# xiaochuanle/MECAT

Measured on AMD Instinct MI355X. Metric: candidate overlaps/sec, higher is better.
Workload: dtype int32

## Files before the change

### mecat_amd/csrc/align.hip

```cpp
#include <stdlib.h>

#include "aln_jobs.h"
#include "dw_defs.h"
#include "scan.h"

__global__ void dw_stitch(const mhip_aln_job* __restrict__ jobs, const DirResult* __restrict__ dres, int n, int min_aln,
                          mhip_aln_result* __restrict__ out, unsigned long long* __restrict__ counters) {
    int i = blockIdx.x * blockDim.x + threadIdx.x;
    if (i >= n) return;
    const DirResult L = dres[2 * i], R = dres[2 * i + 1];
    mhip_aln_result r;
    r.query_start = jobs[i].qstart - L.qbases;
    r.target_start = jobs[i].sstart - L.tbases;
    r.query_end = jobs[i].qstart + R.qbases;
    r.target_end = jobs[i].sstart + R.tbases;
    r.matches = L.matches + R.matches;
    r.columns = L.columns + R.columns;
    r.blocks = L.blocks + R.blocks;
    r.ok = r.columns >= min_aln;
    out[i] = r;
    if (r.ok) {
        atomicAdd(&counters[6], (unsigned long long)(r.query_end - r.query_start));
        atomicAdd(&counters[7], 1ull);
    }
}

__global__ __launch_bounds__(1024) void dw_job_scan(const int32_t* __restrict__ counts, int n_reads, int part_index, int part_count,
                                                    unsigned int* __restrict__ first, int* __restrict__ num_jobs) {
    const unsigned int tot = scan_array_1024<unsigned int>(
        n_reads, 0u, [&](long long i) { return (unsigned int)counts[i]; }, [&](long long i, unsigned int p) { first[i] = p; });
    if (threadIdx.x == 0) {
        unsigned int mine = tot;
        if (part_count > 1) mine = tot / (unsigned)part_count + ((unsigned)part_index < tot % (unsigned)part_count ? 1u : 0u);
        *num_jobs = (int)mine;
    }
}

__global__ __launch_bounds__(256) void dw_make_jobs(const mhip_candidate* __restrict__ cands, const int32_t* __restrict__ counts,
                                                    const unsigned int* __restrict__ first, int n_reads, int maxc, int rid_begin,
                                                    int rid_stride, int ref_start_id, int part_index, int part_count,
                                                    mhip_aln_job* __restrict__ jobs) {
    const size_t t = (size_t)blockIdx.x * blockDim.x + threadIdx.x;
    const int i = (int)(t / (unsigned)maxc), j = (int)(t % (unsigned)maxc);
    if (i >= n_reads || j >= counts[i]) return;
    const unsigned int g = first[i] + (unsigned)j;
    if (part_count > 1 && (int)(g % (unsigned)part_count) != part_index) return;
    const unsigned int slot = part_count > 1 ? g / (unsigned)part_count : g;
    const mhip_candidate cd = cands[(size_t)i * maxc + j];
    mhip_aln_job jb;
    jb.qid_local = rid_begin + i * rid_stride;
    jb.sid_local = cd.readno - ref_start_id;
    jb.chain = cd.chain;
    int qstart = cd.loc2, sstart = cd.loc1;
    if (qstart && sstart) { qstart += MHIP_KMER_SIZE / 2; sstart += MHIP_KMER_SIZE / 2; }
    jb.qstart = qstart;
    jb.sstart = sstart;
    jobs[slot] = jb;
}

int aln_jobs_run(mhip_ctx* c, const mhip_volume* ref, const mhip_volume* reads, const mhip_aln_job* jobs, int n, int min_align_size,
                 mhip_aln_result* out, aln_dev_fn dev) {
    HIPCHK(hipSetDevice(c->device));
    if (n <= 0) return 0;
    char why[96];
    if (aln_jobs_check(jobs, n, reads->h_offs.data(), reads->num_reads, ref->h_offs.data(), ref->num_reads, why, sizeof(why)) >= 0) {
        mhip_set_error("%s", why);
        return -1;
    }
    mhip_aln_job* d_jobs;
    mhip_aln_result* d_out;
    if (c->scratch("al_jobs", sizeof(mhip_aln_job) * (size_t)n, (void**)&d_jobs)) return -1;
    if (c->scratch("al_out", sizeof(mhip_aln_result) * (size_t)n, (void**)&d_out)) return -1;
    HIPCHK(hipMemcpyAsync(d_jobs, jobs, sizeof(mhip_aln_job) * (size_t)n, hipMemcpyHostToDevice, c->stream));
    if (dev(c, ref, reads, d_jobs, n, min_align_size, d_out)) return -1;
    HIPCHK(hipMemcpyAsync(out, d_out, sizeof(mhip_aln_result) * (size_t)n, hipMemcpyDeviceToHost, c->stream));
    HIPCHK(hipStreamSynchronize(c->stream));
    return 0;
}

extern "C" {

int mhip_jobs_from_candidates_dev(mhip_ctx* c, const void* d_cands, const void* d_counts, int n_reads, int maxc, int rid_begin,
                                  int rid_stride, int ref_start_read_id, int part_index, int part_count, void* d_jobs, int* num_jobs) {
    HIPCHK(hipSetDevice(c->device));
    *num_jobs = 0;
    if (n_reads <= 0) return 0;
    if (part_count < 1) part_count = 1;
    int* d_n;
    if (c->scratch("al_njobs", 64, (void**)&d_n)) return -1;
    unsigned int* d_first;
    if (c->scratch("al_jobfirst", sizeof(unsigned int) * (size_t)n_reads, (void**)&d_first)) return -1;
    LAUNCH(c, "dw_job_scan", dw_job_scan, 1, 1024, 0, (const int32_t*)d_counts, n_reads, part_index, part_count, d_first, d_n);
    const size_t nthreads = (size_t)n_reads * (size_t)maxc;
    LAUNCH(c, "dw_make_jobs", dw_make_jobs, (unsigned)((nthreads + 255) / 256), 256, 0, (const mhip_candidate*)d_cands,
           (const int32_t*)d_counts, (const unsigned int*)d_first, n_reads, maxc, rid_begin, rid_stride, ref_start_read_id, part_index,
           part_count, (mhip_aln_job*)d_jobs);
    HIPCHK(hipMemcpyAsync(num_jobs, d_n, sizeof(int), hipMemcpyDeviceToHost, c->stream));
    HIPCHK(hipStreamSynchronize(c->stream));
    return 0;
}

int mhip_align_candidates_dev(mhip_ctx* c, const mhip_volume* ref, const mhip_volume* reads, const void* d_jobs, int n,
                              int min_align_size, void* d_out) {
    HIPCHK(hipSetDevice(c->device));
    if (n <= 0) return 0;
    DirResult* d_dres;
    unsigned int* d_cur;
    if (c->scratch("al_dres", sizeof(DirResult) * 2 * (size_t)n, (void**)&d_dres)) return -1;
    if (c->scratch("al_cursor", 64, (void**)&d_cur)) return -1;
    HIPCHK(hipMemsetAsync(d_cur, 0, 16, c->stream));
    const char* kv = getenv("MECAT_DW_KERNEL");
    if (kv && atoi(kv) == 1) {
        if (dw_extend_launch(c, ref, reads, d_jobs, n, d_dres, nullptr, nullptr, d_cur)) return -1;
    } else {
        DwHandover* d_hand;
        if (c->scratch("al_hand", sizeof(DwHandover) * 2 * (size_t)n, (void**)&d_hand)) return -1;
        if (dw_extend2_launch(c, ref, reads, d_jobs, n, d_dres, d_hand, d_cur + 1, d_cur)) return -1;
        if (dw_extend_launch(c, ref, reads, d_jobs, n, d_dres, d_hand, d_cur + 1, d_cur + 2)) return -1;
    }
    LAUNCH(c, "dw_stitch", dw_stitch, (n + 255) / 256, 256, 0, (const mhip_aln_job*)d_jobs, (const DirResult*)d_dres, n,
           min_align_size, (mhip_aln_result*)d_out, (unsigned long long*)c->d_counters);
    HIPCHK(hipGetLastError());
    return 0;
}

int mhip_align_candidates(mhip_ctx* c, const mhip_volume* ref, const mhip_volume* reads, const mhip_aln_job* jobs, int n,
                          int min_align_size, mhip_aln_result* out) {
    return aln_jobs_run(c, ref, reads, jobs, n, min_align_size, out, mhip_align_candidates_dev);
}

}
```

### mecat_amd/csrc/aln_jobs.h

```cpp
#pragma once
#include <stddef.h>
#include <stdio.h>

#include "mecat_hip.h"

inline int aln_jobs_check(const mhip_aln_job* jobs, int n, const mhip_offset_t* q_offs, int q_reads, const mhip_offset_t* s_offs, int s_reads,
                          char* msg, size_t msg_cap) {
    for (int i = 0; i < n; ++i) {
        const mhip_aln_job& j = jobs[i];
        if (j.qid_local < 0 || j.qid_local >= q_reads || j.sid_local < 0 || j.sid_local >= s_reads) {
            snprintf(msg, msg_cap, "alignment job %d: read index out of range", i);
            return i;
        }
        if (j.qstart > q_offs[(size_t)j.qid_local].size || j.sstart > s_offs[(size_t)j.sid_local].size) {
            snprintf(msg, msg_cap, "alignment job %d: start point outside the reads", i);
            return i;
        }
    }
    return -1;
}

typedef int (*aln_dev_fn)(mhip_ctx* c, const mhip_volume* ref, const mhip_volume* reads, const void* d_jobs, int n, int min_align_size, void* d_out);

int aln_jobs_run(mhip_ctx* c, const mhip_volume* ref, const mhip_volume* reads, const mhip_aln_job* jobs, int n, int min_align_size,
                 mhip_aln_result* out, aln_dev_fn dev);
```

### mecat_amd/csrc/dw_defs.h

```cpp
#pragma once
#include "common.h"

#define AL_BLOCK 256
#define AL_WAVES (AL_BLOCK / WAVE)
#define SEG_BLK 500

struct DirResult {
    int32_t qbases, tbases, matches, columns, blocks, pad;
};

struct DwHandover {
    uint32_t unit;
    int32_t qidx, tidx;
    DirResult R;
};

int dw_extend2_launch(mhip_ctx* c, const mhip_volume* ref, const mhip_volume* reads, const void* d_jobs, int n, DirResult* dres,
                      DwHandover* hand, unsigned int* hand_count, unsigned int* cursor);
int dw_extend_launch(mhip_ctx* c, const mhip_volume* ref, const mhip_volume* reads, const void* d_jobs, int n, DirResult* dres,
                     const DwHandover* hand, const unsigned int* hand_count, unsigned int* cursor);
```

### mecat_amd/csrc/dw_extend.hip

```cpp
#include <stdlib.h>

#include <algorithm>

#include "dw_defs.h"

#define MAX_BLK 736
#define SEQ_WORDS 52
#define MAX_D 400
#define VU_LEN (2 * MAX_D + 8)
#define ROW_W 224
#define RING 16
#define GROW_STRIDE ((size_t)MAX_D * ROW_W + 2 * (MAX_D + 8))

struct AlnWaveLds {
    uint32_t Qp[SEQ_WORDS];
    uint32_t Tp[SEQ_WORDS];
    int16_t V[VU_LEN];
    uint16_t ring[RING * ROW_W];
    int16_t rmin[RING];
    int16_t rmax[RING];
};

#include "dw_helpers.h"

// ... 148 lines not shown
            switch (nj) {
            case 1: row_body<1, SPILL>(S, grow, lane, d, nslot, min_k, max_k, k_offset, q_len, t_len, best_m, band_tol, snake, bkey, hkey, x0); break;
            case 2: row_body<2, SPILL>(S, grow, lane, d, nslot, min_k, max_k, k_offset, q_len, t_len, best_m, band_tol, snake, bkey, hkey, x0); break;
            case 3: row_body<3, SPILL>(S, grow, lane, d, nslot, min_k, max_k, k_offset, q_len, t_len, best_m, band_tol, snake, bkey, hkey, x0); break;
            default: row_body<4, SPILL>(S, grow, lane, d, nslot, min_k, max_k, k_offset, q_len, t_len, best_m, band_tol, snake, bkey, hkey, x0); break;
            }
            xreg = x0;
        }
        bkey = __builtin_amdgcn_readfirstlane(bkey);
        hkey = __builtin_amdgcn_readfirstlane(hkey);
        reg_ok = nj == 1;
        reg_min_k = min_k;
        st.rows += 1; st.fast_rows += fast ? 1u : 0u; st.wide_rows += nj > 1 ? 1u : 0u;
        cells += (unsigned int)nslot;
        {
            const int rm = bkey >> 10, rk = 1023 - (bkey & 1023) - k_offset;
            if (rm > best_m) { best_m = rm; best_x = (rm + rk) / 2; best_y = best_x - rk; best_d = d; best_k = rk; }
        }
        int nmin, nmax;
        bool whole = false;
        if (fast) {
            const int m0 = __builtin_amdgcn_readlane(mreg, 0), ml = __builtin_amdgcn_readlane(mreg, nslot - 1);
            whole = m0 >= best_m - band_tol && ml >= best_m - band_tol;
        }
        if (whole) { nmin = min_k; nmax = max_k; }
        else band_keys<SPILL>(S, lane, nj, nslot, min_k, max_k, k_offset, best_m, band_tol, nmin, nmax);
        max_k = __builtin_amdgcn_readfirstlane(nmax) + 1;
        min_k = __builtin_amdgcn_readfirstlane(nmin) - 1;
        __builtin_amdgcn_wave_barrier();
        if (hkey != 0x7fffffff) {
            aligned = 1; end_k = (hkey >> 10) - k_offset; end_x = hkey & 1023; end_y = end_x - end_k; end_d = d;
            break;
        }
    }
    o.trim_ok = 0; o.qcnt = o.tcnt = o.acnt = 0;
    if (!aligned) {
        st.unaligned += 1;
        if (best_x > 0) { end_x = best_x; end_y = best_y; end_d = best_d; end_k = best_k; }
        else { o.aligned_or_best = 0; o.qe = o.te = o.dist = 0; return; }
    }
    o.aligned_or_best = 1; o.qe = end_x; o.te = end_y; o.dist = end_d;
    const int aln_size = (end_x + end_y + end_d) / 2;
    int cd = end_d, ck = end_k, cx2 = end_x;
    int qcnt = 0, tcnt = 0, acnt = 0, found = 0;
    while (true) {
        int x1, pre_k = 0, takes_q = 0;
        if (cd == 0) x1 = 0;
        else {
            if (!SPILL && last_row - (cd - 1) >= RING) { o.fallback = 1; return; }
            int pmin, pmax, cmin, cmax, vl = 0, vr = 0;
            const int kl = ck - 1, kr = ck + 1;
            if (SPILL) {
                pmin = g_rmin[cd - 1]; pmax = g_rmax[cd - 1]; cmin = g_rmin[cd]; cmax = g_rmax[cd];
                const uint16_t* prow = grow + (size_t)(cd - 1) * ROW_W;
                if (kl >= pmin && kl <= pmax) vl = prow[(kl - pmin) >> 1];
                if (kr >= pmin && kr <= pmax) vr = prow[(kr - pmin) >> 1];
            } else {
                pmin = S.rmin[(cd - 1) % RING]; pmax = S.rmax[(cd - 1) % RING]; cmin = S.rmin[cd % RING]; cmax = S.rmax[cd % RING];
                const uint16_t* prow = S.ring + ((cd - 1) % RING) * ROW_W;
                if (kl >= pmin && kl <= pmax) vl = prow[(kl - pmin) >> 1];
                if (kr >= pmin && kr <= pmax) vr = prow[(kr - pmin) >> 1];
            }
            if (ck == cmin || (ck != cmax && vl < vr)) { x1 = vr; pre_k = kr; takes_q = 0; }
            else { x1 = vl + 1; pre_k = kl; takes_q = 1; }
        }
        const int s = cx2 - x1;
        if (s >= 4) { acnt += 4; qcnt += 4; tcnt += 4; found = 1; break; }
        acnt += s; qcnt += s; tcnt += s;
        if (cd == 0) break;
        acnt += 1;
        if (takes_q) { qcnt += 1; cx2 = x1 - 1; } else { tcnt += 1; cx2 = x1; }
        ck = pre_k;
        --cd;
    }
    o.qcnt = qcnt; o.tcnt = tcnt; o.acnt = acnt;
    o.trim_ok = found && (aln_size - acnt >= 2);
}

__global__ __launch_bounds__(AL_BLOCK) void dw_extend(const uint32_t* __restrict__ rpac, const mhip_offset_t* __restrict__ roffs,
                                                      const uint32_t* __restrict__ qpac, const mhip_offset_t* __restrict__ qoffs,
                                                      const mhip_aln_job* __restrict__ jobs, int n, DirResult* __restrict__ dres,
                                                      uint16_t* __restrict__ gscratch, unsigned int* __restrict__ cursor,
                                                      unsigned long long* __restrict__ counters, const DwHandover* __restrict__ hand,
                                                      const unsigned int* __restrict__ hand_count) {
    __shared__ AlnWaveLds lds[AL_WAVES];
    AlnWaveLds& S = lds[threadIdx.x >> 6];
    const int lane = lane_id();
    const int gw = blockIdx.x * AL_WAVES + (threadIdx.x >> 6);
    uint16_t* grow = gscratch + (size_t)gw * GROW_STRIDE;
    unsigned long long cells = 0, snake = 0, nblocks = 0, nfallback = 0;
    unsigned int ucells = 0, usnake = 0;
    DwStats st = {0, 0, 0, 0, 0};
    while (true) {
        unsigned int unit = 0;
        if (lane == 0) unit = atomicAdd(cursor, 1u);
        unit = __shfl(unit, 0);
        int qidx = 0, tidx = 0;
        DirResult R = {0, 0, 0, 0, 0, 0};
        if (hand) {
            if (unit >= *hand_count) break;
            const DwHandover h = hand[unit];
            unit = h.unit; qidx = h.qidx; tidx = h.tidx; R = h.R;
        } else if (unit >= 2u * (unsigned)n) break;
        const mhip_aln_job jb = jobs[unit >> 1];
        const int right = unit & 1;
        const int qsize = qoffs[jb.qid_local].size, tsize = roffs[jb.sid_local].size;
        SeqView q, t;
        q.pac = qpac; q.off = qoffs[jb.qid_local].offset; q.comp = jb.chain;
        t.pac = rpac; t.off = roffs[jb.sid_local].offset; t.comp = 0;
        int query_size, target_size;
        const int qs0 = right ? jb.qstart : jb.qstart - 1, step = right ? 1 : -1;
        if (jb.chain) { q.A = qsize - 1 - qs0; q.B = -step; } else { q.A = qs0; q.B = step; }
        t.A = right ? jb.sstart : jb.sstart - 1; t.B = step;
        if (right) { query_size = qsize - jb.qstart; target_size = tsize - jb.sstart; }
        else { query_size = jb.qstart; target_size = jb.sstart; }
        if (jb.qstart < 0 || jb.sstart < 0) { query_size = 0; target_size = 0; }
        while (true) {
            const int qleft = query_size - qidx, tleft = target_size - tidx;
            int qblk, tblk, last_block;
            if (qleft < SEG_BLK + 100 || tleft < SEG_BLK + 100) {
                qblk = min(qleft, (int)(tleft + tleft * 0.2));
                tblk = min(tleft, (int)(qleft + qleft * 0.2));
                last_block = 1;
            } else { qblk = SEG_BLK; tblk = SEG_BLK; last_block = 0; }
            if (qblk < 0) qblk = 0;
            if (tblk < 0) tblk = 0;
            __builtin_amdgcn_wave_barrier();
            if (lane < SEQ_WORDS) {
                S.Qp[lane] = (lane > 0 && (lane - 1) * 16 < qblk + 32) ? view_word(q, qidx + (lane - 1) * 16) : 0u;
                S.Tp[lane] = (lane > 0 && (lane - 1) * 16 < tblk + 32) ? view_word(t, tidx + (lane - 1) * 16) : 0u;
            }
            __builtin_amdgcn_wave_barrier();
            BlockOut o;
            align_block<false>(S, qblk, tblk, grow, o, ucells, usnake, st);
            if (o.fallback) { ++nfallback; align_block<true>(S, qblk, tblk, grow, o, ucells, usnake, st); }
            ++nblocks;
            R.blocks += 1;
            if (!o.aligned_or_best || !o.trim_ok) break;
            const int full_map = (qblk - o.qe <= 20 || tblk - o.te <= 20);
            int qcnt = o.qcnt, tcnt = o.tcnt, acnt = o.acnt;
            if (last_block || !full_map) { qcnt -= 4; tcnt -= 4; acnt -= 4; }
            const int cols = (o.qe + o.te + o.dist) / 2 - acnt;
            const int mcut = qcnt + tcnt - acnt;
            R.columns += cols;
            R.matches += (o.qe + o.te - o.dist) / 2 - mcut;
            R.qbases += o.qe - qcnt;
            R.tbases += o.te - tcnt;
            if (last_block || !full_map) break;
            qidx += o.qe - qcnt;
            tidx += o.te - tcnt;
        }
        if (lane == 0) dres[unit] = R;
        cells += ucells; snake += usnake;
        ucells = 0; usnake = 0;
    }
    for (int off = 32; off > 0; off >>= 1) snake += __shfl_xor(snake, off);
    if (lane == 0) {
        atomicAdd(&counters[3], nblocks);
        atomicAdd(&counters[4], cells);
        atomicAdd(&counters[5], snake);
        atomicAdd(&counters[8], nfallback);
        atomicAdd(&counters[9], (unsigned long long)st.rows);
        atomicAdd(&counters[10], (unsigned long long)st.fast_rows);
        atomicAdd(&counters[11], (unsigned long long)st.wide_rows);
        atomicAdd(&counters[12], (unsigned long long)st.unaligned);
    }
}

int dw_extend_launch(mhip_ctx* c, const mhip_volume* ref, const mhip_volume* reads, const void* d_jobs, int n, DirResult* dres,
                     const DwHandover* hand, const unsigned int* hand_count, unsigned int* cursor) {
    int waves_per_cu = 16;
    if (const char* e = getenv("MECAT_DW_WAVES")) waves_per_cu = std::max(4, std::min(32, atoi(e)));
    const int max_waves = c->num_cus * waves_per_cu;
    const int grid = std::min(max_waves / AL_WAVES, (2 * n + AL_WAVES - 1) / AL_WAVES);
    uint16_t* d_g;
    if (c->scratch("al_rows", sizeof(uint16_t) * GROW_STRIDE * (size_t)max_waves, (void**)&d_g)) return -1;
    LAUNCH(c, "dw_extend", dw_extend, grid, AL_BLOCK, 0, (const uint32_t*)ref->d_pac, (const mhip_offset_t*)ref->d_offs,
           (const uint32_t*)reads->d_pac, (const mhip_offset_t*)reads->d_offs, (const mhip_aln_job*)d_jobs, n, dres, d_g, cursor,
           (unsigned long long*)c->d_counters, hand, hand_count);
    return 0;
}
```

### mecat_amd/csrc/xalign.hip

```cpp
#include <stdlib.h>

#include <algorithm>
#include <type_traits>

#include "aln_jobs.h"
#include "common.h"
#include "xd_defs.h"
#include "xd_block_ring.h"
#include "xd_block_wide.h"

template <bool WIDE>
__global__ __launch_bounds__(XW_BLOCK, 6) void xd_extend_w(const uint32_t* __restrict__ rpac, const mhip_offset_t* __restrict__ roffs,
                                                        const uint32_t* __restrict__ qpac, const mhip_offset_t* __restrict__ qoffs,
                                                        const mhip_aln_job* __restrict__ jobs, int n, XDir* __restrict__ dres,
                                                        uint8_t* __restrict__ scratch, unsigned int* __restrict__ cursor,
                                                        unsigned int* __restrict__ ovf_list, unsigned long long* __restrict__ counters,
                                                        const unsigned int* __restrict__ ulist, unsigned int nunits,
                                                        uint8_t* __restrict__ wide_state, const unsigned int* __restrict__ order) {
    __shared__ typename std::conditional<WIDE, XwWide, XrLds>::type lds[WIDE ? 1 : XW_WAVES];
    auto& S = lds[threadIdx.x >> 6];
    const int lane = lane_id();
    uint8_t* st = scratch + (size_t)(blockIdx.x * (blockDim.x >> 6) + (threadIdx.x >> 6)) * (WIDE ? XW_WIDE_BYTES : XR_STATE_BYTES);
    uint8_t* wst = WIDE ? nullptr : wide_state + (size_t)(blockIdx.x * (blockDim.x >> 6) + (threadIdx.x >> 6)) * XW_INPLACE_BYTES;
    unsigned long long nblocks = 0, ncells = 0, nrows = 0, nredone = 0;
// ... 107 lines not shown
    mhip_aln_result r;
    r.query_start = jobs[i].qstart - L.qbases;
    r.target_start = jobs[i].sstart - L.tbases;
    r.query_end = jobs[i].qstart + R.qbases;
    r.target_end = jobs[i].sstart + R.tbases;
    r.matches = L.matches + R.matches;
    r.columns = L.columns + R.columns;
    r.blocks = L.blocks + R.blocks;
    r.ok = (r.query_end - r.query_start) >= min_aln;
    out[i] = r;
    if (r.ok) {
        atomicAdd(&counters[6], (unsigned long long)(r.query_end - r.query_start));
        atomicAdd(&counters[7], 1ull);
    }
}

struct XdMode {
    bool all_wide;
    bool handover;
    bool order;
    int waves_per_cu;
};
static XdMode xd_mode() {
    auto is = [](const char* name, int v) { const char* s = getenv(name); return s && atoi(s) == v; };
    XdMode m;
    m.all_wide = is("MECAT_XD_WIDE", 1);
    m.handover = is("MECAT_XD_HANDOVER", 1);
    m.order = !is("MECAT_XD_ORDER", 0);
    m.waves_per_cu = getenv("MECAT_XW_WAVES") ? atoi(getenv("MECAT_XW_WAVES")) : 24;
    return m;
}

static int xd_launch_ring(mhip_ctx* c, const mhip_volume* ref, const mhip_volume* reads, const void* d_jobs, int n, bool handover, int waves,
                          XDir* d_dres, unsigned int* d_cur, unsigned int* d_ovf, const unsigned int* d_order, unsigned int* nwide) {
    const int grid = std::min(waves / XW_WAVES, (2 * n + XW_WAVES - 1) / XW_WAVES);
    const size_t launched = (size_t)grid * XW_WAVES;
    uint8_t *d_s, *d_wst = nullptr;
    if (c->scratch("xw_state", XR_STATE_BYTES * launched, (void**)&d_s)) return -1;
    if (!handover && c->scratch("xw_inplace", XW_INPLACE_BYTES * launched, (void**)&d_wst)) return -1;
    LAUNCH(c, "xd_extend_w", xd_extend_w<false>, grid, XW_BLOCK, 0, (const uint32_t*)ref->d_pac, (const mhip_offset_t*)ref->d_offs,
           (const uint32_t*)reads->d_pac, (const mhip_offset_t*)reads->d_offs, (const mhip_aln_job*)d_jobs, n, d_dres, d_s, d_cur,
           d_ovf, (unsigned long long*)c->d_counters, (const unsigned int*)nullptr, 2u * (unsigned)n, d_wst, d_order);
    HIPCHK(hipMemcpyAsync(nwide, d_ovf, sizeof(unsigned int), hipMemcpyDeviceToHost, c->stream));
    HIPCHK(hipStreamSynchronize(c->stream));
    if (getenv("MECAT_TRACE")) {
        if (d_wst) {
            unsigned long long redone = 0;
            HIPCHK(hipMemcpy(&redone, (unsigned long long*)c->d_counters + 33, sizeof(redone), hipMemcpyDeviceToHost));
            fprintf(stderr, "[mecat_hip] X-drop: %d units, %llu blocks so far redone in place with the wide window\n", 2 * n, redone);
        } else fprintf(stderr, "[mecat_hip] X-drop: %u of %d units need the wide-window path\n", *nwide, 2 * n);
    }
    return 0;
}

static int xd_launch_wide(mhip_ctx* c, const mhip_volume* ref, const mhip_volume* reads, const void* d_jobs, int n, XDir* d_dres,
                          unsigned int* d_cur, unsigned int* d_ovf, const unsigned int* ulist, unsigned int nu) {
    const int wgrid = (int)std::min(nu, 2048u);
    uint8_t* d_w;
    if (c->scratch("xw_wide", XW_WIDE_BYTES * (size_t)wgrid, (void**)&d_w)) return -1;
    LAUNCH(c, "xd_extend_wide", xd_extend_w<true>, wgrid, 64, 0, (const uint32_t*)ref->d_pac, (const mhip_offset_t*)ref->d_offs,
           (const uint32_t*)reads->d_pac, (const mhip_offset_t*)reads->d_offs, (const mhip_aln_job*)d_jobs, n, d_dres, d_w, d_cur + 2,
           d_ovf + 6 * (size_t)n + 4, (unsigned long long*)c->d_counters, ulist, nu, (uint8_t*)nullptr, (const unsigned int*)nullptr);
    return 0;
}

extern "C" {

int mhip_xalign_candidates_dev(mhip_ctx* c, const mhip_volume* ref, const mhip_volume* reads, const void* d_jobs, int n,
                               int min_align_size, void* d_out) {
    HIPCHK(hipSetDevice(c->device));
    if (n <= 0) return 0;
    const XdMode mode = xd_mode();
    XDir* d_dres;
    unsigned int *d_cur, *d_ovf;
    if (c->scratch("xa_dres", sizeof(XDir) * 2 * (size_t)n, (void**)&d_dres)) return -1;
    if (c->scratch("xa_cursor", 64, (void**)&d_cur)) return -1;
    if (c->scratch("xa_ovf", sizeof(unsigned int) * (6 * (size_t)n + 8), (void**)&d_ovf)) return -1;
    HIPCHK(hipMemsetAsync(d_cur, 0, 16, c->stream));
    unsigned int nwide = 0;
    if (!mode.all_wide) {
        const int waves = c->num_cus * mode.waves_per_cu;
        HIPCHK(hipMemsetAsync(d_ovf, 0, sizeof(unsigned int), c->stream));
        unsigned int* d_order = nullptr;
        if (mode.order && xd_order_jobs(c, ref, reads, d_jobs, n, waves, &d_order)) return -1;
        if (xd_launch_ring(c, ref, reads, d_jobs, n, mode.handover, waves, d_dres, d_cur, d_ovf, d_order, &nwide)) return -1;
    }
    if (nwide > 0 || mode.all_wide) {
        const unsigned int* ulist = mode.all_wide ? nullptr : d_ovf + 1;
        if (xd_launch_wide(c, ref, reads, d_jobs, n, d_dres, d_cur, d_ovf, ulist, mode.all_wide ? 2u * (unsigned)n : nwide)) return -1;
    }
    LAUNCH(c, "xd_stitch", xd_stitch, (n + 255) / 256, 256, 0, (const mhip_aln_job*)d_jobs, (const XDir*)d_dres, n, min_align_size,
           (mhip_aln_result*)d_out, (unsigned long long*)c->d_counters);
    HIPCHK(hipStreamSynchronize(c->stream));
    HIPCHK(hipGetLastError());
    return 0;
}

int mhip_xalign_candidates(mhip_ctx* c, const mhip_volume* ref, const mhip_volume* reads, const mhip_aln_job* jobs, int n,
                           int min_align_size, mhip_aln_result* out) {
    return aln_jobs_run(c, ref, reads, jobs, n, min_align_size, out, mhip_xalign_candidates_dev);
}

}
```

### mecat_amd/csrc/xd_defs.h

```cpp
#pragma once
#include "common.h"

#define X_SEG 500
#define X_MAXN 736
#define X_MIN_SCORE (-100000000)

enum { XS_SUB = 3, XS_GAP_IN_A = 0, XS_GAP_IN_B = 6, XS_OP_MASK = 0x07, XS_EXT_A = 0x10, XS_EXT_B = 0x40 };

struct XDir {
    int32_t qbases, tbases, matches, columns;
    int32_t last_q, last_t, last_m;
    int32_t blocks;
};

struct XView {
    const uint32_t* pac;
    int64_t off;
    int A, B, comp;
};
__device__ __forceinline__ int xv_at(const XView& v, int i) {
    const uint32_t c = pac_base(v.pac, v.off + v.A + (int64_t)v.B * i);
    return (int)(v.comp ? 3u - c : c);
}

// ... 32 lines not shown
    int m = 0, found = 0;
    int want_l1 = 0, first = 0, l1 = 0;
    int sn_n = 0, sn_a = 0, sn_b = 0, sn_m = 0;

    __device__ __forceinline__ void column_type(int pk) {
        first = n == 0 ? pk : first;
        l1 = want_l1 ? pk : l1;
        want_l1 = 0;
    }
    __device__ __forceinline__ void step(int cq, int ct, int cm, int a_after, int b_after) {
        column_type(cq | (ct << 1) | (cm << 2));
        ++n;
        nmatch += cm;
        m = cm ? m + 1 : 0;
        if (m == 4 && !found) { found = 1; want_l1 = 1; sn_n = n; sn_a = a_after; sn_b = b_after; sn_m = nmatch; }
    }
    __device__ __forceinline__ void run(int r, uint32_t Mbits, int a_before, int b_before) {
        const uint32_t mask = r >= 32 ? 0xffffffffu : ((1u << r) - 1u);
        const uint32_t inv = ~Mbits & mask;
        if (!found) {
            const int z = inv ? __builtin_ctz(inv) : r;
            int hit = -1;
            if (m + z >= 4) hit = 3 - m;
            else {
                const uint32_t Q = Mbits & (Mbits >> 1) & (Mbits >> 2) & (Mbits >> 3);
                if (Q) hit = __builtin_ctz(Q) + 3;
            }
            if (hit >= 0) {
                found = 1;
                sn_n = n + hit + 1; sn_a = a_before - (hit + 1); sn_b = b_before - (hit + 1);
                sn_m = nmatch + __builtin_popcount(Mbits & ((2u << hit) - 1u));
                if (hit + 1 < r) l1 = 3 | (int)(((Mbits >> (hit + 1)) & 1u) << 2);
                else want_l1 = 1;
            }
        }
        m = inv ? r - 1 - (31 - __builtin_clz(inv)) : m + r;
    }
    __device__ __forceinline__ void gap_after_run(int gq, int gt) {
        l1 = want_l1 ? (gq | (gt << 1)) : l1;
        want_l1 = 0;
        m = 0;
        ++n;
    }
    __device__ __forceinline__ void finish(int ae, int be, XBlockOut& o) const {
        o.n = n; o.nmatch = nmatch;
        o.l0q = first & 1; o.l0t = (first >> 1) & 1; o.l0m = first >> 2;
        o.l1q = l1 & 1; o.l1t = (l1 >> 1) & 1; o.l1m = l1 >> 2;
        o.acnt = found ? sn_n : n; o.qcnt = found ? ae - sn_a : ae; o.tcnt = found ? be - sn_b : be; o.mtail = found ? sn_m : nmatch;
        o.trim_ok = found && (n - o.acnt >= 2);
    }
};

#define XW_WAVES 4
#define XW_BLOCK (XW_WAVES * 64)
#define XW_RING 128
#define XW_ROWCELLS 128
#define XW_WIN 4096
#define XW_WSTRIDE 768
#define XW_WIDE_BYTES ((size_t)(X_MAXN + 2) * XW_WSTRIDE)
#define XW_WIDE_HF (X_MAXN + 8)
#define XW_INPLACE_STATE 16384
#define XW_INPLACE_BYTES (XW_INPLACE_STATE + XW_WIDE_BYTES)
#define XW_NEG (-(1 << 30))
#define XS_MATCH 0x80
static_assert(XW_ROWCELLS <= XW_RING, "a row's script cells are cells of the ring");
static_assert(XW_WSTRIDE >= X_MAXN + 1 && XW_WIDE_HF >= X_MAXN + 1, "a wide row and the wide score array hold every cell of a block");
static_assert(XW_WIN % 256 == 0, "the wide traceback's window is loaded in rounds of one dword per lane");

template <int CTRL, int RMASK> __device__ __forceinline__ int xw_dpp_max(int v) {
    return max(v, __builtin_amdgcn_update_dpp((int)0x80000000, v, CTRL, RMASK, 0xf, false));
}
__device__ __forceinline__ int xw_scan_max(int v) {
    v = xw_dpp_max<0x111, 0xf>(v);
    v = xw_dpp_max<0x112, 0xf>(v);
    v = xw_dpp_max<0x114, 0xf>(v);
    v = xw_dpp_max<0x118, 0xf>(v);
    v = xw_dpp_max<0x142, 0xa>(v);
    v = xw_dpp_max<0x143, 0xc>(v);
    return v;
}
__device__ __forceinline__ int xw_shr1(int v, int fill) {
    return __builtin_amdgcn_update_dpp(fill, v, 0x138, 0xf, 0xf, false);
}

int xd_order_jobs(mhip_ctx* c, const mhip_volume* ref, const mhip_volume* reads, const void* d_jobs, int n, int waves, unsigned int** d_order);
```

### mecat_amd/csrc/xd_order.hip

```cpp
#include <algorithm>

#include "common.h"
#include "scan.h"
#include "xd_defs.h"

#define XO_BINS 64
__device__ __forceinline__ int xo_bin(const mhip_aln_job& jb, const mhip_offset_t* __restrict__ roffs, const mhip_offset_t* __restrict__ qoffs) {
    int reach = 0;
    if (jb.qstart >= 0 && jb.sstart >= 0) {
        const int qsize = qoffs[jb.qid_local].size, tsize = roffs[jb.sid_local].size;
        reach = max(min(qsize - jb.qstart, tsize - jb.sstart), min(jb.qstart, jb.sstart));
    }
    return XO_BINS - 1 - min(max(reach, 0) >> 10, XO_BINS - 1);
}
#define XO_THREADS 256
template <bool PLACE>
__global__ __launch_bounds__(XO_THREADS) void xo_order_jobs(const mhip_aln_job* __restrict__ jobs, int n, const mhip_offset_t* __restrict__ roffs,
                                                          const mhip_offset_t* __restrict__ qoffs, unsigned int* __restrict__ cnt, unsigned int* __restrict__ order) {
    __shared__ uint16_t tc[XO_BINS][XO_THREADS];
    __shared__ unsigned int wsum[XO_THREADS / 64];
    __shared__ unsigned int base;
    const int t = (int)threadIdx.x, G = (int)gridDim.x;
    const int per_block = (n + G - 1) / G, b0 = min(n, (int)blockIdx.x * per_block), b1 = min(n, b0 + per_block);
    const int per = (b1 - b0 + XO_THREADS - 1) / XO_THREADS, lo = min(b1, b0 + t * per), hi = min(b1, lo + per);
    for (int b = 0; b < XO_BINS; ++b) tc[b][t] = 0;
    for (int i = lo; i < hi; ++i) ++tc[xo_bin(jobs[i], roffs, qoffs)][t];
    __syncthreads();
    unsigned int mypos[XO_BINS];
#pragma unroll
    for (int b = 0; b < XO_BINS; ++b) {
        if (t == 0) base = PLACE ? cnt[(size_t)b * G + blockIdx.x] : 0u;
        const unsigned int c = tc[b][t];
        unsigned int incl = c;
        for (int o = 1; o < 64; o <<= 1) {
            const unsigned int v = __shfl_up(incl, o);
            if ((t & 63) >= o) incl += v;
        }
        if ((t & 63) == 63) wsum[t >> 6] = incl;
        __syncthreads();
        unsigned int before = base;
        for (int k = 0; k < (t >> 6); ++k) before += wsum[k];
        mypos[b] = before + incl - c;
        if (!PLACE && t == XO_THREADS - 1) cnt[(size_t)b * G + blockIdx.x] = before + incl;
        __syncthreads();
    }
    if (!PLACE) return;
    for (int i = lo; i < hi; ++i) {
        const int b = xo_bin(jobs[i], roffs, qoffs);
        unsigned int p = 0;
#pragma unroll
        for (int k = 0; k < XO_BINS; ++k) if (k == b) p = mypos[k]++;
        order[p] = (unsigned int)i;
    }
}
__global__ __launch_bounds__(1024) void xo_scan(unsigned int* __restrict__ cnt, int m) {
    scan_array_1024<unsigned int>(m, 0u, [&](long long i) { return cnt[i]; }, [&](long long i, unsigned int p) { cnt[i] = p; });
}

int xd_order_jobs(mhip_ctx* c, const mhip_volume* ref, const mhip_volume* reads, const void* d_jobs, int n, int waves, unsigned int** d_order) {
    *d_order = nullptr;
    if ((size_t)n <= (size_t)waves) return 0;
    const int G = (int)std::min<size_t>((size_t)c->num_cus, ((size_t)n + 4095) / 4096 + 1);
    unsigned int *d_cnt, *d_ord;
    if (c->scratch("xo_cnt", sizeof(unsigned int) * XO_BINS * (size_t)G, (void**)&d_cnt)) return -1;
    if (c->scratch("xo_order", sizeof(unsigned int) * (size_t)n, (void**)&d_ord)) return -1;
    if ((size_t)n / ((size_t)G * XO_THREADS) >= 65535) return 0;
    LAUNCH(c, "xo_count", xo_order_jobs<false>, G, XO_THREADS, 0, (const mhip_aln_job*)d_jobs, n, (const mhip_offset_t*)ref->d_offs, (const mhip_offset_t*)reads->d_offs, d_cnt, d_ord);
    LAUNCH(c, "xo_scan", xo_scan, 1, 1024, 0, d_cnt, XO_BINS * G);
    LAUNCH(c, "xo_place", xo_order_jobs<true>, G, XO_THREADS, 0, (const mhip_aln_job*)d_jobs, n, (const mhip_offset_t*)ref->d_offs, (const mhip_offset_t*)reads->d_offs, d_cnt, d_ord);
    *d_order = d_ord;
    return 0;
}
```

Measured before the change: 7.067 million.

## Order DW jobs and handover units longest-first and run handover blocks directly

Reuses the xd binning sort, moved to a shared file, to reorder alignment jobs by estimated reach, longest first. The jobs are permuted before the two-stage extend kernels, and results are scattered back to the original order in stitch. The handover units for the second kernel are also bin-sorted by remaining distance in a single-block kernel. Handover blocks now skip the fast-path attempt and go straight to the full-row alignment. The aim is to cut tail imbalance across waves and avoid redundant fast-path attempts that would fall back anyway, at the cost of extra sort and permute kernels.

```diff
diff --git a/mecat_amd/csrc/align.hip b/mecat_amd/csrc/align.hip
--- a/mecat_amd/csrc/align.hip
+++ b/mecat_amd/csrc/align.hip
@@ -1,11 +1,19 @@
 #include <stdlib.h>
+
+#include <algorithm>
 
 #include "aln_jobs.h"
 #include "dw_defs.h"
 #include "scan.h"
 
+__global__ void dw_permute_jobs(const mhip_aln_job* __restrict__ jobs, const unsigned int* __restrict__ order, int n,
+                                mhip_aln_job* __restrict__ ordered) {
+    const int p = blockIdx.x * blockDim.x + threadIdx.x;
+    if (p < n) ordered[p] = jobs[order[p]];
+}
+
 __global__ void dw_stitch(const mhip_aln_job* __restrict__ jobs, const DirResult* __restrict__ dres, int n, int min_aln,
-                          mhip_aln_result* __restrict__ out, unsigned long long* __restrict__ counters) {
+                          mhip_aln_result* __restrict__ out, unsigned long long* __restrict__ counters, const unsigned int* __restrict__ order) {
     int i = blockIdx.x * blockDim.x + threadIdx.x;
     if (i >= n) return;
     const DirResult L = dres[2 * i], R = dres[2 * i + 1];
@@ -18,7 +26,7 @@
     r.columns = L.columns + R.columns;
     r.blocks = L.blocks + R.blocks;
     r.ok = r.columns >= min_aln;
-    out[i] = r;
+    out[order ? order[i] : (unsigned int)i] = r;
     if (r.ok) {
         atomicAdd(&counters[6], (unsigned long long)(r.query_end - r.query_start));
         atomicAdd(&counters[7], 1ull);
@@ -110,16 +118,28 @@
     if (c->scratch("al_cursor", 64, (void**)&d_cur)) return -1;
     HIPCHK(hipMemsetAsync(d_cur, 0, 16, c->stream));
     const char* kv = getenv("MECAT_DW_KERNEL");
+    unsigned int* d_order = nullptr;
     if (kv && atoi(kv) == 1) {
-        if (dw_extend_launch(c, ref, reads, d_jobs, n, d_dres, nullptr, nullptr, d_cur)) return -1;
+        if (dw_extend_launch(c, ref, reads, d_jobs, n, d_dres, nullptr, nullptr, d_cur, nullptr)) return -1;
     } else {
         DwHandover* d_hand;
         if (c->scratch("al_hand", sizeof(DwHandover) * 2 * (size_t)n, (void**)&d_hand)) return -1;
+        const char* ov = getenv("MECAT_DW_ORDER");
+        const int order_mode = ov ? atoi(ov) : 1;
+        int waves_per_cu = DW2_WAVES_PER_SIMD * 4;
+        if (const char* e = getenv("MECAT_DW_WAVES")) waves_per_cu = std::max(4, std::min(32, atoi(e)));
+        if (order_mode != 0 && aln_order_jobs(c, ref, reads, d_jobs, n, order_mode == 2 ? 0 : c->num_cus * waves_per_cu, &d_order)) return -1;
+        if (d_order) {
+            mhip_aln_job* d_ordered;
+            if (c->scratch("al_jobs_ordered", sizeof(mhip_aln_job) * (size_t)n, (void**)&d_ordered)) return -1;
+            LAUNCH(c, "dw_permute_jobs", dw_permute_jobs, (n + 255) / 256, 256, 0, (const mhip_aln_job*)d_jobs, (const unsigned int*)d_order, n, d_ordered);
+            d_jobs = d_ordered;
+        }
         if (dw_extend2_launch(c, ref, reads, d_jobs, n, d_dres, d_hand, d_cur + 1, d_cur)) return -1;
-        if (dw_extend_launch(c, ref, reads, d_jobs, n, d_dres, d_hand, d_cur + 1, d_cur + 2)) return -1;
+        if (dw_extend_launch(c, ref, reads, d_jobs, n, d_dres, d_hand, d_cur + 1, d_cur + 2, d_cur + 3)) return -1;
     }
     LAUNCH(c, "dw_stitch", dw_stitch, (n + 255) / 256, 256, 0, (const mhip_aln_job*)d_jobs, (const DirResult*)d_dres, n,
-           min_align_size, (mhip_aln_result*)d_out, (unsigned long long*)c->d_counters);
+           min_align_size, (mhip_aln_result*)d_out, (unsigned long long*)c->d_counters, (const unsigned int*)d_order);
     HIPCHK(hipGetLastError());
     return 0;
 }
diff --git a/mecat_amd/csrc/aln_jobs.h b/mecat_amd/csrc/aln_jobs.h
--- a/mecat_amd/csrc/aln_jobs.h
+++ b/mecat_amd/csrc/aln_jobs.h
@@ -20,6 +20,8 @@
     return -1;
 }
 
+int aln_order_jobs(mhip_ctx* c, const mhip_volume* ref, const mhip_volume* reads, const void* d_jobs, int n, int waves, unsigned int** d_order);
+
 typedef int (*aln_dev_fn)(mhip_ctx* c, const mhip_volume* ref, const mhip_volume* reads, const void* d_jobs, int n, int min_align_size, void* d_out);
 
 int aln_jobs_run(mhip_ctx* c, const mhip_volume* ref, const mhip_volume* reads, const mhip_aln_job* jobs, int n, int min_align_size,
diff --git a/mecat_amd/csrc/aln_order.hip b/mecat_amd/csrc/aln_order.hip
--- /dev/null
+++ b/mecat_amd/csrc/aln_order.hip
@@ -0,0 +1,73 @@
+#include <algorithm>
+
+#include "aln_jobs.h"
+#include "common.h"
+#include "scan.h"
+
+#define XO_BINS 64
+__device__ __forceinline__ int xo_bin(const mhip_aln_job& jb, const mhip_offset_t* __restrict__ roffs, const mhip_offset_t* __restrict__ qoffs) {
+    int reach = 0;
+    if (jb.qstart >= 0 && jb.sstart >= 0) {
+        const int qsize = qoffs[jb.qid_local].size, tsize = roffs[jb.sid_local].size;
+        reach = max(min(qsize - jb.qstart, tsize - jb.sstart), min(jb.qstart, jb.sstart));
+    }
+    return XO_BINS - 1 - min(max(reach, 0) >> 10, XO_BINS - 1);
+}
+#define XO_THREADS 256
+template <bool PLACE>
+__global__ __launch_bounds__(XO_THREADS) void xo_order_jobs(const mhip_aln_job* __restrict__ jobs, int n, const mhip_offset_t* __restrict__ roffs,
+                                                          const mhip_offset_t* __restrict__ qoffs, unsigned int* __restrict__ cnt, unsigned int* __restrict__ order) {
+    __shared__ uint16_t tc[XO_BINS][XO_THREADS];
+    __shared__ unsigned int wsum[XO_THREADS / 64];
+    __shared__ unsigned int base;
+    const int t = (int)threadIdx.x, G = (int)gridDim.x;
+    const int per_block = (n + G - 1) / G, b0 = min(n, (int)blockIdx.x * per_block), b1 = min(n, b0 + per_block);
+    const int per = (b1 - b0 + XO_THREADS - 1) / XO_THREADS, lo = min(b1, b0 + t * per), hi = min(b1, lo + per);
+    for (int b = 0; b < XO_BINS; ++b) tc[b][t] = 0;
+    for (int i = lo; i < hi; ++i) ++tc[xo_bin(jobs[i], roffs, qoffs)][t];
+    __syncthreads();
+    unsigned int mypos[XO_BINS];
+#pragma unroll
+    for (int b = 0; b < XO_BINS; ++b) {
+        if (t == 0) base = PLACE ? cnt[(size_t)b * G + blockIdx.x] : 0u;
+        const unsigned int c = tc[b][t];
+        unsigned int incl = c;
+        for (int o = 1; o < 64; o <<= 1) {
+            const unsigned int v = __shfl_up(incl, o);
+            if ((t & 63) >= o) incl += v;
+        }
+        if ((t & 63) == 63) wsum[t >> 6] = incl;
+        __syncthreads();
+        unsigned int before = base;
+        for (int k = 0; k < (t >> 6); ++k) before += wsum[k];
+        mypos[b] = before + incl - c;
+        if (!PLACE && t == XO_THREADS - 1) cnt[(size_t)b * G + blockIdx.x] = before + incl;
+        __syncthreads();
+    }
+    if (!PLACE) return;
+    for (int i = lo; i < hi; ++i) {
+        const int b = xo_bin(jobs[i], roffs, qoffs);
+        unsigned int p = 0;
+#pragma unroll
+        for (int k = 0; k < XO_BINS; ++k) if (k == b) p = mypos[k]++;
+        order[p] = (unsigned int)i;
+    }
+}
+__global__ __launch_bounds__(1024) void xo_scan(unsigned int* __restrict__ cnt, int m) {
+    scan_array_1024<unsigned int>(m, 0u, [&](long long i) { return cnt[i]; }, [&](long long i, unsigned int p) { cnt[i] = p; });
+}
+
+int aln_order_jobs(mhip_ctx* c, const mhip_volume* ref, const mhip_volume* reads, const void* d_jobs, int n, int waves, unsigned int** d_order) {
+    *d_order = nullptr;
+    if ((size_t)n <= (size_t)waves) return 0;
+    const int G = (int)std::min<size_t>((size_t)c->num_cus, ((size_t)n + 4095) / 4096 + 1);
+    unsigned int *d_cnt, *d_ord;
+    if (c->scratch("xo_cnt", sizeof(unsigned int) * XO_BINS * (size_t)G, (void**)&d_cnt)) return -1;
+    if (c->scratch("xo_order", sizeof(unsigned int) * (size_t)n, (void**)&d_ord)) return -1;
+    if ((size_t)n / ((size_t)G * XO_THREADS) >= 65535) return 0;
+    LAUNCH(c, "xo_count", xo_order_jobs<false>, G, XO_THREADS, 0, (const mhip_aln_job*)d_jobs, n, (const mhip_offset_t*)ref->d_offs, (const mhip_offset_t*)reads->d_offs, d_cnt, d_ord);
+    LAUNCH(c, "xo_scan", xo_scan, 1, 1024, 0, d_cnt, XO_BINS * G);
+    LAUNCH(c, "xo_place", xo_order_jobs<true>, G, XO_THREADS, 0, (const mhip_aln_job*)d_jobs, n, (const mhip_offset_t*)ref->d_offs, (const mhip_offset_t*)reads->d_offs, d_cnt, d_ord);
+    *d_order = d_ord;
+    return 0;
+}
diff --git a/mecat_amd/csrc/dw_defs.h b/mecat_amd/csrc/dw_defs.h
--- a/mecat_amd/csrc/dw_defs.h
+++ b/mecat_amd/csrc/dw_defs.h
@@ -17,5 +17,12 @@
 
 int dw_extend2_launch(mhip_ctx* c, const mhip_volume* ref, const mhip_volume* reads, const void* d_jobs, int n, DirResult* dres,
                       DwHandover* hand, unsigned int* hand_count, unsigned int* cursor);
+#ifndef DW2_WAVES_PER_SIMD
+#define DW2_WAVES_PER_SIMD 8
+#endif
 int dw_extend_launch(mhip_ctx* c, const mhip_volume* ref, const mhip_volume* reads, const void* d_jobs, int n, DirResult* dres,
-                     const DwHandover* hand, const unsigned int* hand_count, unsigned int* cursor);
+                     const DwHandover* hand, const unsigned int* hand_count, unsigned int* cursor, unsigned int* hand_sorted);
+
+#define DW_SLOT_RERUN 46
+#define DW_SLOT_DIRECT 47
+#define DW_SLOT_DEALT 48
diff --git a/mecat_amd/csrc/dw_extend.hip b/mecat_amd/csrc/dw_extend.hip
--- a/mecat_amd/csrc/dw_extend.hip
+++ b/mecat_amd/csrc/dw_extend.hip
@@ -254,13 +254,14 @@
                                                       const mhip_aln_job* __restrict__ jobs, int n, DirResult* __restrict__ dres,
                                                       uint16_t* __restrict__ gscratch, unsigned int* __restrict__ cursor,
                                                       unsigned long long* __restrict__ counters, const DwHandover* __restrict__ hand,
-                                                      const unsigned int* __restrict__ hand_count) {
+                                                      const unsigned int* __restrict__ hand_count, const unsigned int* __restrict__ hand_order,
+                                                      const unsigned int* __restrict__ hand_sorted, int hand_direct) {
     __shared__ AlnWaveLds lds[AL_WAVES];
     AlnWaveLds& S = lds[threadIdx.x >> 6];
     const int lane = lane_id();
     const int gw = blockIdx.x * AL_WAVES + (threadIdx.x >> 6);
     uint16_t* grow = gscratch + (size_t)gw * GROW_STRIDE;
-    unsigned long long cells = 0, snake = 0, nblocks = 0, nfallback = 0;
+    unsigned long long cells = 0, snake = 0, nblocks = 0, nfallback = 0, ndirect = 0, ndealt = 0;
     unsigned int ucells = 0, usnake = 0;
     DwStats st = {0, 0, 0, 0, 0};
     while (true) {
@@ -269,10 +270,14 @@
         unit = __shfl(unit, 0);
         int qidx = 0, tidx = 0;
         DirResult R = {0, 0, 0, 0, 0, 0};
+        bool keep_rows = false;
         if (hand) {
             if (unit >= *hand_count) break;
-            const DwHandover h = hand[unit];
+            const bool sorted = *hand_sorted != 0u;
+            const DwHandover h = hand[sorted ? hand_order[unit] : unit];
+            ndealt += sorted ? 1u : 0u;
             unit = h.unit; qidx = h.qidx; tidx = h.tidx; R = h.R;
+            keep_rows = hand_direct != 0;
         } else if (unit >= 2u * (unsigned)n) break;
         const mhip_aln_job jb = jobs[unit >> 1];
         const int right = unit & 1;
@@ -304,8 +309,13 @@
             }
             __builtin_amdgcn_wave_barrier();
             BlockOut o;
-            align_block<false>(S, qblk, tblk, grow, o, ucells, usnake, st);
-            if (o.fallback) { ++nfallback; align_block<true>(S, qblk, tblk, grow, o, ucells, usnake, st); }
+            if (keep_rows) ++ndirect;
+            else {
+                align_block<false>(S, qblk, tblk, grow, o, ucells, usnake, st);
+                if (o.fallback) { ++nfallback; keep_rows = true; }
+            }
+            if (keep_rows) align_block<true>(S, qblk, tblk, grow, o, ucells, usnake, st);
+            keep_rows = false;
             ++nblocks;
             R.blocks += 1;
             if (!o.aligned_or_best || !o.trim_ok) break;
@@ -331,7 +341,9 @@
         atomicAdd(&counters[3], nblocks);
         atomicAdd(&counters[4], cells);
         atomicAdd(&counters[5], snake);
-        atomicAdd(&counters[8], nfallback);
+        atomicAdd(&counters[DW_SLOT_RERUN], nfallback);
+        atomicAdd(&counters[DW_SLOT_DIRECT], ndirect);
+        atomicAdd(&counters[DW_SLOT_DEALT], ndealt);
         atomicAdd(&counters[9], (unsigned long long)st.rows);
         atomicAdd(&counters[10], (unsigned long long)st.fast_rows);
         atomicAdd(&counters[11], (unsigned long long)st.wide_rows);
@@ -339,16 +351,91 @@
     }
 }
 
+#define HO_BINS 64
+#define HO_THREADS 256
+#define HO_MAX 65536
+__global__ __launch_bounds__(HO_THREADS) void dw_hand_order(const DwHandover* __restrict__ hand, const unsigned int* __restrict__ hand_count,
+                                                            const mhip_aln_job* __restrict__ jobs, const mhip_offset_t* __restrict__ roffs,
+                                                            const mhip_offset_t* __restrict__ qoffs, unsigned int max_sorted,
+                                                            uint8_t* __restrict__ keys, unsigned int* __restrict__ order,
+                                                            unsigned int* __restrict__ sorted) {
+    __shared__ uint16_t tc[HO_BINS][HO_THREADS];
+    __shared__ unsigned int bin_first[HO_BINS];
+    const unsigned int cnt = *hand_count;
+    if (cnt < 2u || cnt > max_sorted) return;
+    const int t = (int)threadIdx.x, w = t >> 6, l = t & 63;
+    for (int b = 0; b < HO_BINS; ++b) tc[b][t] = 0;
+#pragma unroll 4
+    for (unsigned int i = t; i < cnt; i += HO_THREADS) {
+        const unsigned int unit = hand[i].unit;
+        const int qidx = hand[i].qidx, tidx = hand[i].tidx;
+        const mhip_aln_job jb = jobs[unit >> 1];
+        int rest = 0;
+        if (jb.qstart >= 0 && jb.sstart >= 0) {
+            const int qsize = qoffs[jb.qid_local].size, tsize = roffs[jb.sid_local].size;
+            rest = (unit & 1u) ? min(qsize - jb.qstart - qidx, tsize - jb.sstart - tidx) : min(jb.qstart - qidx, jb.sstart - tidx);
+        }
+        const int b = HO_BINS - 1 - min(max(rest, 0) >> 10, HO_BINS - 1);
+        keys[i] = (uint8_t)b;
+    }
+    __syncthreads();
+    const unsigned int per = (cnt + HO_THREADS - 1) / HO_THREADS, lo = min(cnt, t * per), hi = min(cnt, lo + per);
+    for (unsigned int i = lo; i < hi; ++i) ++tc[keys[i]][t];
+    __syncthreads();
+    for (int b = w; b < HO_BINS; b += HO_THREADS / 64) {
+        unsigned int c[4], sum = 0;
+        for (int k = 0; k < 4; ++k) { c[k] = tc[b][4 * l + k]; sum += c[k]; }
+        unsigned int incl = sum;
+        for (int o = 1; o < 64; o <<= 1) {
+            const unsigned int v = __shfl_up(incl, o);
+            if (l >= o) incl += v;
+        }
+        unsigned int before = incl - sum;
+        for (int k = 0; k < 4; ++k) { tc[b][4 * l + k] = (uint16_t)before; before += c[k]; }
+        if (l == 63) bin_first[b] = incl;
+    }
+    __syncthreads();
+    if (t < HO_BINS) {
+        const unsigned int cb = bin_first[t];
+        unsigned int incl = cb;
+        for (int o = 1; o < 64; o <<= 1) {
+            const unsigned int v = __shfl_up(incl, o);
+            if (l >= o) incl += v;
+        }
+        bin_first[t] = incl - cb;
+    }
+    __syncthreads();
+    for (unsigned int i = lo; i < hi; ++i) {
+        const int b = keys[i];
+        order[bin_first[b] + tc[b][t]++] = i;
+    }
+    if (t == 0) *sorted = 1u;
+}
+
 int dw_extend_launch(mhip_ctx* c, const mhip_volume* ref, const mhip_volume* reads, const void* d_jobs, int n, DirResult* dres,
-                     const DwHandover* hand, const unsigned int* hand_count, unsigned int* cursor) {
+                     const DwHandover* hand, const unsigned int* hand_count, unsigned int* cursor, unsigned int* hand_sorted) {
     int waves_per_cu = 16;
     if (const char* e = getenv("MECAT_DW_WAVES")) waves_per_cu = std::max(4, std::min(32, atoi(e)));
     const int max_waves = c->num_cus * waves_per_cu;
     const int grid = std::min(max_waves / AL_WAVES, (2 * n + AL_WAVES - 1) / AL_WAVES);
     uint16_t* d_g;
     if (c->scratch("al_rows", sizeof(uint16_t) * GROW_STRIDE * (size_t)max_waves, (void**)&d_g)) return -1;
+    const char* e = getenv("MECAT_DW_HAND_DIRECT");
+    const int hand_direct = hand && !(e && atoi(e) == 0);
+    unsigned int* d_ord = nullptr;
+    if (hand) {
+        e = getenv("MECAT_DW_HAND_SORT_MAX");
+        const size_t max_sorted = std::min<size_t>(e ? (size_t)std::max(0, atoi(e)) : (size_t)HO_MAX, (size_t)HO_MAX);
+        const size_t cap = std::max<size_t>(std::min<size_t>(2 * (size_t)n, max_sorted), 1);
+        uint8_t* d_keys;
+        if (c->scratch("al_handord", sizeof(unsigned int) * cap, (void**)&d_ord)) return -1;
+        if (c->scratch("al_handkey", cap, (void**)&d_keys)) return -1;
+        if (max_sorted >= 2)
+            LAUNCH(c, "dw_hand_order", dw_hand_order, 1, HO_THREADS, 0, hand, hand_count, (const mhip_aln_job*)d_jobs,
+                   (const mhip_offset_t*)ref->d_offs, (const mhip_offset_t*)reads->d_offs, (unsigned int)max_sorted, d_keys, d_ord, hand_sorted);
+    }
     LAUNCH(c, "dw_extend", dw_extend, grid, AL_BLOCK, 0, (const uint32_t*)ref->d_pac, (const mhip_offset_t*)ref->d_offs,
            (const uint32_t*)reads->d_pac, (const mhip_offset_t*)reads->d_offs, (const mhip_aln_job*)d_jobs, n, dres, d_g, cursor,
-           (unsigned long long*)c->d_counters, hand, hand_count);
+           (unsigned long long*)c->d_counters, hand, hand_count, (const unsigned int*)d_ord, (const unsigned int*)hand_sorted, hand_direct);
     return 0;
 }
diff --git a/mecat_amd/csrc/xalign.hip b/mecat_amd/csrc/xalign.hip
--- a/mecat_amd/csrc/xalign.hip
+++ b/mecat_amd/csrc/xalign.hip
@@ -213,7 +213,7 @@
         const int waves = c->num_cus * mode.waves_per_cu;
         HIPCHK(hipMemsetAsync(d_ovf, 0, sizeof(unsigned int), c->stream));
         unsigned int* d_order = nullptr;
-        if (mode.order && xd_order_jobs(c, ref, reads, d_jobs, n, waves, &d_order)) return -1;
+        if (mode.order && aln_order_jobs(c, ref, reads, d_jobs, n, waves, &d_order)) return -1;
         if (xd_launch_ring(c, ref, reads, d_jobs, n, mode.handover, waves, d_dres, d_cur, d_ovf, d_order, &nwide)) return -1;
     }
     if (nwide > 0 || mode.all_wide) {
diff --git a/mecat_amd/csrc/xd_defs.h b/mecat_amd/csrc/xd_defs.h
--- a/mecat_amd/csrc/xd_defs.h
+++ b/mecat_amd/csrc/xd_defs.h
@@ -138,5 +138,3 @@
 __device__ __forceinline__ int xw_shr1(int v, int fill) {
     return __builtin_amdgcn_update_dpp(fill, v, 0x138, 0xf, 0xf, false);
 }
-
-int xd_order_jobs(mhip_ctx* c, const mhip_volume* ref, const mhip_volume* reads, const void* d_jobs, int n, int waves, unsigned int** d_order);
diff --git a/mecat_amd/csrc/xd_order.hip b/mecat_amd/csrc/xd_order.hip
--- a/mecat_amd/csrc/xd_order.hip
+++ /dev/null
@@ -1,73 +0,0 @@
-#include <algorithm>
-
-#include "common.h"
-#include "scan.h"
-#include "xd_defs.h"
-
-#define XO_BINS 64
-__device__ __forceinline__ int xo_bin(const mhip_aln_job& jb, const mhip_offset_t* __restrict__ roffs, const mhip_offset_t* __restrict__ qoffs) {
-    int reach = 0;
-    if (jb.qstart >= 0 && jb.sstart >= 0) {
-        const int qsize = qoffs[jb.qid_local].size, tsize = roffs[jb.sid_local].size;
-        reach = max(min(qsize - jb.qstart, tsize - jb.sstart), min(jb.qstart, jb.sstart));
-    }
-    return XO_BINS - 1 - min(max(reach, 0) >> 10, XO_BINS - 1);
-}
-#define XO_THREADS 256
-template <bool PLACE>
-__global__ __launch_bounds__(XO_THREADS) void xo_order_jobs(const mhip_aln_job* __restrict__ jobs, int n, const mhip_offset_t* __restrict__ roffs,
-                                                          const mhip_offset_t* __restrict__ qoffs, unsigned int* __restrict__ cnt, unsigned int* __restrict__ order) {
-    __shared__ uint16_t tc[XO_BINS][XO_THREADS];
-    __shared__ unsigned int wsum[XO_THREADS / 64];
-    __shared__ unsigned int base;
-    const int t = (int)threadIdx.x, G = (int)gridDim.x;
-    const int per_block = (n + G - 1) / G, b0 = min(n, (int)blockIdx.x * per_block), b1 = min(n, b0 + per_block);
-    const int per = (b1 - b0 + XO_THREADS - 1) / XO_THREADS, lo = min(b1, b0 + t * per), hi = min(b1, lo + per);
-    for (int b = 0; b < XO_BINS; ++b) tc[b][t] = 0;
-    for (int i = lo; i < hi; ++i) ++tc[xo_bin(jobs[i], roffs, qoffs)][t];
-    __syncthreads();
-    unsigned int mypos[XO_BINS];
-#pragma unroll
-    for (int b = 0; b < XO_BINS; ++b) {
-        if (t == 0) base = PLACE ? cnt[(size_t)b * G + blockIdx.x] : 0u;
-        const unsigned int c = tc[b][t];
-        unsigned int incl = c;
-        for (int o = 1; o < 64; o <<= 1) {
-            const unsigned int v = __shfl_up(incl, o);
-            if ((t & 63) >= o) incl += v;
-        }
-        if ((t & 63) == 63) wsum[t >> 6] = incl;
-        __syncthreads();
-        unsigned int before = base;
-        for (int k = 0; k < (t >> 6); ++k) before += wsum[k];
-        mypos[b] = before + incl - c;
-        if (!PLACE && t == XO_THREADS - 1) cnt[(size_t)b * G + blockIdx.x] = before + incl;
-        __syncthreads();
-    }
-    if (!PLACE) return;
-    for (int i = lo; i < hi; ++i) {
-        const int b = xo_bin(jobs[i], roffs, qoffs);
-        unsigned int p = 0;
-#pragma unroll
-        for (int k = 0; k < XO_BINS; ++k) if (k == b) p = mypos[k]++;
-        order[p] = (unsigned int)i;
-    }
-}
-__global__ __launch_bounds__(1024) void xo_scan(unsigned int* __restrict__ cnt, int m) {
-    scan_array_1024<unsigned int>(m, 0u, [&](long long i) { return cnt[i]; }, [&](long long i, unsigned int p) { cnt[i] = p; });
-}
-
-int xd_order_jobs(mhip_ctx* c, const mhip_volume* ref, const mhip_volume* reads, const void* d_jobs, int n, int waves, unsigned int** d_order) {
-    *d_order = nullptr;
-    if ((size_t)n <= (size_t)waves) return 0;
-    const int G = (int)std::min<size_t>((size_t)c->num_cus, ((size_t)n + 4095) / 4096 + 1);
-    unsigned int *d_cnt, *d_ord;
-    if (c->scratch("xo_cnt", sizeof(unsigned int) * XO_BINS * (size_t)G, (void**)&d_cnt)) return -1;
-    if (c->scratch("xo_order", sizeof(unsigned int) * (size_t)n, (void**)&d_ord)) return -1;
-    if ((size_t)n / ((size_t)G * XO_THREADS) >= 65535) return 0;
-    LAUNCH(c, "xo_count", xo_order_jobs<false>, G, XO_THREADS, 0, (const mhip_aln_job*)d_jobs, n, (const mhip_offset_t*)ref->d_offs, (const mhip_offset_t*)reads->d_offs, d_cnt, d_ord);
-    LAUNCH(c, "xo_scan", xo_scan, 1, 1024, 0, d_cnt, XO_BINS * G);
-    LAUNCH(c, "xo_place", xo_order_jobs<true>, G, XO_THREADS, 0, (const mhip_aln_job*)d_jobs, n, (const mhip_offset_t*)ref->d_offs, (const mhip_offset_t*)reads->d_offs, d_cnt, d_ord);
-    *d_order = d_ord;
-    return 0;
-}
```

Result: no change. 7.128 million (median of 6 runs) (+0.9%).
